# fuxiao0719/PanopticNeRF

Hardware: AMD Instinct MI355X
Metric: Msamples/sec (coarse+fine), KITTI-360 1408x376 (higher is better)
Workload: dtype bf16

## Files before the change

panopticnerf_amd/csrc/asm/gen_mlp_tt.py:

```python
#!/usr/bin/env python3
import os
import sys

if os.path.dirname(os.path.abspath(__file__)) not in sys.path:
    sys.path.insert(0, os.path.dirname(os.path.abspath(__file__)))
import tt_math
import tt_plan
from tt_emit import Emitter
from tt_regs import *



def vr(lo, n):
    return "v[%d:%d]" % (lo, lo + n - 1) if n > 1 else "v%d" % lo


def ar(lo, n):
    return "a[%d:%d]" % (lo, lo + n - 1) if n > 1 else "a%d" % lo


def sr(lo, n=2):
    return "s[%d:%d]" % (lo, lo + n - 1) if n > 1 else "s%d" % lo


# ... 26 lines not shown
        self.NC = len(self.chunks)
        self.units = tt_plan.build_units(self.layers, self.chunks)
        self.stream = []
        for u in self.units:
            u["frag0"] = len(self.stream)
            self.stream += [(sl, of) for sl, of, _, _ in self.unit_frags(u)]

    def unit_frags(self, u):
        return tt_plan.unit_frags(self.layers, self.chunks, u)

    def chunk_base(self, chunk):
        self.e("s_add_u32 s%d, s%d, 0x%x" % (S_PIECE, S_IMG, self.chunks[chunk]["off"] * 1024))
        self.e("s_addc_u32 s%d, s%d, 0" % (S_PIECE + 1, S_IMG + 1))

    def piece(self, chunk, j):
        m, i, nw = tt_plan.piece_list(self.chunks, chunk)[j]
        slot = chunk % NSLOT
        skip = None
        certain = nw >= 4
        if not certain:
            skip = self.label()
            self.e("s_cmp_ge_u32 s%d, %d" % (S_WAVE, nw))
            self.e("s_cbranch_scc1 %s" % skip)
        m0 = slot * SLOT + 16 * m * 1024
        if self.m0 != m0 or skip or self.trace:
            self.e("s_add_u32 m0, s%d, 0x%x" % (S_W4K, m0))
            self.e("s_nop 0")
        self.m0 = None if skip else m0
        tag = self.vm_op("global_load_lds_dwordx4 v%d, s[%d:%d] offset:%d" % (V_DMA + m, S_PIECE, S_PIECE + 1, i * 1024), certain)
        if skip:
            self.o.append(skip + ":")
        return tag

    def issue_piece(self, chunk, j):
        if j == 0:
            self.chunk_base(chunk)
        self.piece_tag[chunk] = self.piece(chunk, j)

    def hand_over(self, chunk):
        if not self.abl & 2:
            self.wait_vm(self.piece_tag.get((chunk + 2) % self.NC))
            self.e("s_barrier")

    def loc_of(self, seg, layer_index, t, ks):
        if seg == "ex":
            return Loc("v", V_EX + 16 * t + 4 * ks)
        if seg == "ed":
            return Loc("v", V_ED + 8 * t + 4 * ks)
        if seg == "h":
            src = self.trunk_out(layer_index - 1)
            return Loc("a", src + 64 * t + 4 * ks)
        if seg == "tap":
            return Loc("a", (self.F_base() if self.tap else self.trunk_out(D - 1)) + 64 * t + 4 * ks)
        if seg == "hh":
            return Loc("a", self.trunk_out(D - 1) + 64 * t + 4 * ks)
        if seg == "F":
            return Loc("a", self.F_base() + 64 * t + 4 * ks)
# ... 243 lines not shown

    def acc_reg(self, i):
        return V_ACC + 16 * i

    def acc_take(self, n):
        assert len(self.acc_free) >= n, ("accumulators exhausted", self.acc_free)
        got, self.acc_free = self.acc_free[:n], self.acc_free[n:]
        return got

    def acc_release(self, ids):
        self.acc_free = sorted(set(self.acc_free) | set(ids))

    def arm_plan(self, u):
        c = self.chunks[u["chunk"]]
        l = self.layers[u["layer"]]
        slot = u["chunk"] % NSLOT
        bias_off = c["nfb"] * l["nks"] * 1024
        u["accs"], u["arm_tags"] = {}, []
        plans = []
        for bi, blk in enumerate(u["blocks"]):
            b_in_chunk = blk - c["fb"]
            for t in range(2):
                key = (bi, t)
                ops = []

                def take(key=key):
                    while not self.acc_free and self.side_busy():
                        self.drain_side(8)
                    u["accs"][key] = self.acc_take(1)[0]
                if t == 1:
                    plans.append([take])
                    continue
                if l["mode"] == "logits":
                    def first(key=key, slot=slot, take=take):
                        take()
                        self.e("v_add_u32 v%d, 0x%x, v%d" % (self.acc_reg(u["accs"][key]), slot * SLOT, V_LB4))
                    ops.append(first)
                    for r in list(range(1, 16)) + [0]:
                        ops.append(lambda key=key, r=r, off=bias_off + b_in_chunk * 128: u["arm_tags"].append(
                            self.lgkm_op("ds_read_b32 v%d, v%d offset:%d" % (self.acc_reg(u["accs"][key]) + r, self.acc_reg(u["accs"][key]), off))))
                else:
                    for m in range(4):
                        def rd(key=key, m=m, off=bias_off + b_in_chunk * 128 + m * 32, take=take):
                            if m == 0:
                                take()
                            a = self.acc_reg(u["accs"][key])
                            u["arm_tags"].append(self.lgkm_op("ds_read_b128 %s, v%d offset:%d" % (vr(a + 4 * m, 4), V_BIAS + slot, off)))
                        ops.append(rd)
                plans.append(ops)
        return plans

    def pack_ops(self, u):
        l = self.layers[u["layer"]]
        if not self.trace:
            return self.pack_ops_pipelined(u)
        out = []
        for bi, blk in enumerate(u["blocks"]):
            for t in range(2):
                a = self.acc_reg(u["accs"][(bi, t)])
                dst = self.out_block(l, blk, t)
                for p in range(8):
                    def fn(a=a, p=p, dst=dst, relu=(l["mode"] == "relu"), k=len(out)):
# ... 312 lines not shown
                        a = self.acc_reg(u["accs"][(bi, t)])
                        dst = self.sm_sums[t][kk]
                        if r == 0:
                            e("v_fma_f32 v%d, v%d, v%d, 0" % (dst, M[t], a))
                        else:
                            e("v_fmac_f32 v%d, v%d, v%d" % (dst, M[t] + r, a + r))

    def lwr_ops(self):
        ops = []

        def first():
            while self.side or self.outbox or (len(self.acc_free) < 2 and self.side_busy()):
                self.drain_side(8)
            assert len(self.acc_free) >= 2, ("no free accumulators for the local weights", self.acc_free)
            self.lwr_acc = self.acc_take(2)
            self.e("v_add_u32 v%d, s%d, v%d" % (V_LWA, S_LWR, V_BIAS + 0))
        ops.append(first)
        for t in range(2):
            for q in range(4):
                for h2 in range(2):
                    def rd(t=t, q=q, h2=h2):
                        dst = self.acc_reg(self.lwr_acc[t]) + 4 * q + ((2 * h2 + 2) & 3)
                        self.lwr_tag = self.lgkm_op("ds_read_b64 %s, v%d offset:%d" % (vr(dst, 2), V_LWA, 128 * t + 32 * q + 8 * h2))
                    ops.append(rd)
        return ops

    def logit_blocks(self):
        return [(b, False) for b in range(self.nbs)] + [(0, True)] * self.nbi

    def tail_logits(self):
        e = self.e
# ... 135 lines not shown
        assert self.acc_free == [i for i in range(8) if i not in self.units[0]["accs"].values()], self.acc_free
        self.last_stamp = None
        for ui in range(len(self.units)):
            self.emit_unit(ui)
        self.stamp(len(self.units))
        self.drain_side()
        self.tail_logits()
        self.stamp(len(self.units) + 1)
        assert self.acc_free == list(range(8)), self.acc_free
        self.e("s_waitcnt lgkmcnt(0)")
        self.lgkm.drain()
        self.advance_group_state()
        self.stamp(len(self.units) + 2)
        if self.trace:
            self.o.append("\ts_waitcnt lgkmcnt(0)")
            self.stamp(len(self.units) + 3)

    def kernel(self):
        e, name = self.e, self.name
        self.o += ["\t.text", "\t.globl\t%s" % name, "\t.p2align\t8", "\t.type\t%s,@function" % name, "%s:" % name]
        for dst, off, n in ((S_IMG, 0x0, 2), (S_RAYS, 0x8, 2), (S_Z, 0x10, 2), (S_S, 0x18, 2), (S_MAGIC, 0x20, 2), (S_NGRP, 0x28, 2),
                            (S_REC, 0x30, 2), (S_RECF, 0x38, 1), (S_PS, 0x40, 2), (S_NSEM, 0x48, 2), (S_CLK, 0x50, 2), (S_AUX, 0x58, 2)):
            e("s_load_dword%s %s, %s, 0x%x" % ("x2" if n == 2 else "", sr(dst, n), sr(S_KARG), off))
        e("v_readfirstlane_b32 s%d, v0" % S_WAVE)
        e("s_nop 4")
        e("s_lshr_b32 s%d, s%d, 6" % (S_WAVE, S_WAVE))
        e("s_lshl_b32 s%d, s%d, 12" % (S_W4K, S_WAVE))
        e("v_and_b32 v%d, 63, v0" % V_T0)
        e("v_lshlrev_b32 v%d, 4, v%d" % (V_LANE16, V_T0))
        e("v_lshrrev_b32 v%d, 5, v0" % V_LB4)
        e("v_and_b32 v%d, 1, v%d" % (V_LB4, V_LB4))
        e("v_lshlrev_b32 v%d, 4, v%d" % (V_LB4, V_LB4))
        for sl in range(NSLOT):
            self.lit(S_T0, sl * SLOT)
            e("v_add_u32 v%d, s%d, v%d" % (V_FRAG + sl, S_T0, V_LANE16))
            e("v_add_u32 v%d, s%d, v%d" % (V_BIAS + sl, S_T0, V_LB4))
        for k in range(3):
            e("v_add_u32 v%d, s%d, v%d" % (V_DMA + k, S_W4K, V_LANE16))
            if k:
                e("v_add_u32 v%d, 0x%x, v%d" % (V_DMA + k, 16384 * k, V_DMA + k))
        e("v_and_b32 v%d, 31, v0" % V_LB4)
        e("v_lshlrev_b32 v%d, 2, v%d" % (V_LB4, V_LB4))
        e("s_mov_b32 s%d, -1" % S_LO32)
        e("s_mov_b32 s%d, 0" % (S_LO32 + 1))
        e("s_mov_b32 s%d, 1" % S_N0)
        e("s_mov_b32 s%d, 1" % (S_N0 + 1))
        e("s_mov_b32 s%d, -1" % S_HI0)
        e("s_mov_b32 s%d, 0" % (S_HI0 + 1))
        e("s_lshr_b32 s%d, s%d, 4" % (S_LWW, S_W4K))
        e("s_add_u32 s%d, s%d, 0x%x" % (S_LWW, S_LWW, LW_BASE))
        e("s_sub_u32 s%d, s%d, 0x%x" % (S_LWR, S_LWW, 0))
        e("s_waitcnt lgkmcnt(0)")
        for k, (blk, inst) in enumerate(self.logit_blocks()):
            e("v_and_b32 v%d, 31, v0" % V_T0)
            if blk:
                e("v_add_u32 v%d, %d, v%d" % (V_T0, 32 * blk, V_T0))
            e("v_cmp_gt_i32 vcc, s%d, v%d" % (S_NINST if inst else S_NSEM, V_T0))
            e("s_and_b64 s[%d:%d], vcc, s[%d:%d]" % (S_MSK + 2 * k, S_MSK + 2 * k + 1, S_HI0, S_HI0 + 1))
        if self.softmax:
            for k, (nblk, sreg) in enumerate(((self.nbs, S_NSEM), (self.nbi, S_NINST))):
                if nblk:
                    e("v_and_b32 v%d, 31, v0" % V_T0)
                    if nblk > 1:
                        e("v_add_u32 v%d, %d, v%d" % (V_T0, 32 * (nblk - 1), V_T0))
                    e("v_cmp_gt_i32 s[%d:%d], s%d, v%d" % (S_VMSK + 2 * k, S_VMSK + 2 * k + 1, sreg, V_T0))
        lend, lloop, lfin = self.label(), self.label(), self.label()
        e("s_mov_b32 s%d, s%d" % (S_GRP, S_WG))
        e("s_cmp_ge_i32 s%d, s%d" % (S_GRP, S_NGRP))
        e("s_cbranch_scc1 %s" % lend)
        for c in range(3):
            for j in range(tt_plan.pieces_of(self.chunks, c)):
                self.issue_piece(c, j)
        e("s_waitcnt vmcnt(0)")
        self.vm.drain()
        e("s_barrier")
        e("s_mov_b32 s%d, s%d" % (S_GRP2, S_GRP))
        tags = [self.fetch_tile(t, S_GRP2) for t in range(2)]
        for t in range(2):
            self.wait_vm(tags[t])
            for part in ("x", "d"):
                for fn in self.encode_tile(t, part):
                    fn()
        self.advance_group_state()
        if not self.trace:
            e("s_memtime s[%d:%d]" % (S_CLK0, S_CLK0 + 1))
            e("s_memrealtime s[%d:%d]" % (S_CLK0 + 2, S_CLK0 + 3))
        else:
            e("v_mov_b32 v%d, 0" % V_TRACE)
            e("s_mov_b32 s%d, 0" % S_NDONE)
            e("s_memtime %s" % sr(S_WGCLK))
            e("s_waitcnt lgkmcnt(0)")
        e("s_waitcnt lgkmcnt(0)")
        self.lgkm.drain()
        self.prefetch_first_unit()
        keep = self.o
        self.o = []
        self.group_body()
        self.prefetch_first_unit()
        self.o = keep
        self.o.append(lloop + ":")
        self.group_body()
        e("s_add_u32 s%d, s%d, s%d" % (S_GRP, S_GRP, S_NWG))
        e("s_cmp_ge_i32 s%d, s%d" % (S_GRP, S_NGRP))
        e("s_cbranch_scc1 %s" % lend)
# ... 10 lines not shown
            e("s_memtime s[%d:%d]" % (S_CLK0, S_CLK0 + 1))
            e("s_waitcnt lgkmcnt(0)")
            e("s_sub_u32 s%d, s%d, s%d" % (S_CLK0, S_CLK0, S_WGCLK))
            e("s_lshl_b32 s%d, s%d, 2" % (S_T0, S_WG))
            e("s_add_u32 s%d, s%d, 256" % (S_T0, S_T0))
            e("v_mov_b32 v%d, s%d" % (V_T0, S_T0))
            e("v_mov_b32 v%d, s%d" % (V_T1, S_CLK0))
            e("s_mov_b64 exec, 1")
            e("global_store_dword v%d, v%d, s[%d:%d]" % (V_T0, V_T1, S_CLK, S_CLK + 1))
            e("s_mov_b64 exec, -1")
            e("s_waitcnt vmcnt(0)")
            self.o.append(lw + ":")
        e("s_cmp_lg_u32 s%d, 0" % S_WG)
        e("s_cbranch_scc1 %s" % lfin)
        if self.trace:
            e("s_cmp_lg_u32 s%d, 0" % S_WAVE)
            e("s_cbranch_scc1 %s" % lfin)
            e("v_and_b32 v%d, 63, v0" % V_T0)
            e("v_lshlrev_b32 v%d, 2, v%d" % (V_T0, V_T0))
            e("global_store_dword v%d, v%d, s[%d:%d]" % (V_T0, V_TRACE, S_CLK, S_CLK + 1))
            e("s_waitcnt vmcnt(0)")
            e("s_branch %s" % lfin)
        e("s_memtime s[%d:%d]" % (S_T0, S_T0 + 1))
        e("s_memrealtime s[%d:%d]" % (S_SAVE, S_SAVE + 1))
        e("s_waitcnt lgkmcnt(0)")
        e("s_sub_u32 s%d, s%d, s%d" % (S_T0, S_T0, S_CLK0))
        e("s_subb_u32 s%d, s%d, s%d" % (S_T1, S_T1, S_CLK0 + 1))
        e("s_sub_u32 s%d, s%d, s%d" % (S_SAVE, S_SAVE, S_CLK0 + 2))
        e("s_subb_u32 s%d, s%d, s%d" % (S_SAVE + 1, S_SAVE + 1, S_CLK0 + 3))
        e("v_cmp_eq_u32 vcc, 0, v0")
        e("s_and_saveexec_b64 s[%d:%d], vcc" % (S_VALID, S_VALID + 1))
        e("s_cbranch_execz %s" % lfin)
        e("v_mov_b32 v%d, s%d" % (V_CLKOUT, S_T0))
        e("v_mov_b32 v%d, s%d" % (V_CLKOUT + 1, S_T1))
        e("v_mov_b32 v%d, s%d" % (V_CLKOUT + 2, S_SAVE))
        e("v_mov_b32 v%d, s%d" % (V_CLKOUT + 3, S_SAVE + 1))
        e("v_mov_b32 v%d, 0" % V_T0)
        e("global_store_dwordx4 v%d, %s, s[%d:%d]" % (V_T0, vr(V_CLKOUT, 4), S_CLK, S_CLK + 1))
        e("s_waitcnt vmcnt(0)")
        self.o.append(lfin + ":")
        e("s_endpgm")
        self.o += [".Lend_%s:" % name, "\t.size\t%s, .Lend_%s-%s" % (name, name, name), ""]
        self.o += ["\t.rodata", "\t.p2align\t6", "\t.amdhsa_kernel %s" % name,
                   "\t\t.amdhsa_group_segment_fixed_size %d" % (NSLOT * SLOT + 1024),
                   "\t\t.amdhsa_private_segment_fixed_size 0", "\t\t.amdhsa_kernarg_size %d" % KERNARG_BYTES, "\t\t.amdhsa_user_sgpr_count 2",
                   "\t\t.amdhsa_user_sgpr_kernarg_segment_ptr 1", "\t\t.amdhsa_system_sgpr_workgroup_id_x 1",
                   "\t\t.amdhsa_system_vgpr_workitem_id 0", "\t\t.amdhsa_next_free_vgpr 512", "\t\t.amdhsa_next_free_sgpr %d" % NEXT_FREE_SGPR,
                   "\t\t.amdhsa_accum_offset 256", "\t\t.amdhsa_reserve_vcc 1", "\t\t.amdhsa_float_denorm_mode_32 3",
                   "\t\t.amdhsa_float_denorm_mode_16_64 3", "\t\t.amdhsa_dx10_clamp 1", "\t\t.amdhsa_ieee_mode 1",
                   "\t.end_amdhsa_kernel", ""]
        return "\n".join(self.o)


KERNARG_BYTES = 104


def metadata(names):
    o = ["\t.amdgpu_metadata", "---", "amdhsa.kernels:"]
    for n in names:
        o += ["  - .agpr_count:     256", "    .args:", "      - .offset:         0", "        .size:           %d" % KERNARG_BYTES,
              "        .value_kind:     by_value", "    .group_segment_fixed_size: %d" % (NSLOT * SLOT + 1024),
              "    .kernarg_segment_align: 8", "    .kernarg_segment_size: %d" % KERNARG_BYTES, "    .max_flat_workgroup_size: 256",
              "    .name:           %s" % n, "    .private_segment_fixed_size: 0", "    .sgpr_count:     108",
              "    .sgpr_spill_count: 0", "    .symbol:         %s.kd" % n, "    .uniform_work_group_size: 1",
              "    .uses_dynamic_stack: false", "    .vgpr_count:     512", "    .vgpr_spill_count: 0", "    .wavefront_size: 64"]
    o += ["amdhsa.target:   amdgcn-amd-amdhsa--gfx950", "amdhsa.version:", "  - 1", "  - 2", "...", "\t.end_amdgpu_metadata", ""]
    return "\n".join(o)


def variant_name(tap, depth, sm, nbs, nbi):
    tag = ("f" if tap else "") + ("d1" if depth == 1 else "") + ("sm" if sm else "")
    return "k_mlp_tt_%ss%di%d" % (tag + "_" if tag else "", nbs, nbi)


def main():
    out = sys.argv[1] if len(sys.argv) > 1 else "/dev/stdout"
    parts = ['\t.amdgcn_target "amdgcn-amd-amdhsa--gfx950"', "\t.amdhsa_code_object_version 5", ""]
    names = []
    for nbs, nbi in ((1, 1), (2, 1), (0, 0), (1, 0), (2, 0), (3, 0)):
        n = "k_mlp_tt_s%di%d" % (nbs, nbi)
        names.append(n)
        parts.append(Gen(nbs, nbi, n).kernel())
    for tap in (0, 1):
        for depth in (2, 1):
            for sm in (False, True):
                if (tap, depth, sm) == (0, 2, False):
                    continue
                for nbs, nbi in ((1, 1), (2, 1), (1, 0), (2, 0), (3, 0)):
                    n = variant_name(tap, depth, sm, nbs, nbi)
                    names.append(n)
                    parts.append(Gen(nbs, nbi, n, depth=depth, softmax=sm, tap=tap).kernel())
    extra = sys.argv[3] if len(sys.argv) > 3 else ""
    if extra in ("trace", "abl"):
        names.append("k_mlp_tt_s2i1_trace")
        parts.append(Gen(2, 1, "k_mlp_tt_s2i1_trace", trace=True).kernel())
    if extra == "abl":
        for abl in (1, 2, 3, 4, 7):
            names.append("k_mlp_tt_s2i1_trace_a%d" % abl)
            parts.append(Gen(2, 1, names[-1], trace=True, abl=abl).kernel())
    unit_names = ["%s %s" % (g.layers[u["layer"]]["name"], u["blocks"]) for g in [Gen(2, 1, "x")] for u in g.units]
    if len(sys.argv) > 2:
        open(sys.argv[2], "w").write("\n".join(unit_names) + "\n")
    parts.append(metadata(names))
    with open(out, "w") as f:
        f.write("\n".join(parts))


if __name__ == "__main__":
    main()
```

panopticnerf_amd/csrc/asm/tt_plan.py:

```python
from tt_regs import D, NSLOT, SKIP


def build_plan(nbs, nbi, depth):
    L = []

    def add(name, nblk, segs, fbc, mode):
        nks = sum(n for _, n in segs)
        if fbc * nks + 1 > 33:
            fbc = 1
        L.append(dict(name=name, nblk=nblk, segs=segs, nks=nks, fbc=fbc, mode=mode))
    for i in range(D):
        if i == 0:
            add("L0", 8, [("ex", 4)], 8, "relu")
        elif i - 1 == SKIP:
            add("L%d" % i, 8, [("ex", 4), ("h", 16)], 2, "relu")
        else:
            add("L%d" % i, 8, [("h", 16)], 2, "relu")
    add("feature", 8, [("h", 16)], 2, "linear")
    add("views", 4, [("F", 16), ("ed", 2)], 2, "relu")
    add("rgbs", 1, [("g", 8), ("hh", 16)], 1, "rgbs")
    if depth == 1:
        if nbs:
            add("sem1", nbs, [("tap", 16)], nbs, "logits")
        if nbi:
            add("inst1", 1, [("tap", 16)], 1, "logits")
    else:
        if nbs:
            add("sem0", 4, [("tap", 16)], 2, "relu")
        if nbi:
            add("inst0", 4, [("tap", 16)], 2, "relu")
        if nbs:
            add("sem1", nbs, [("shs", 8)], nbs, "logits")
        if nbi:
            add("inst1", 1, [("shi", 8)], 1, "logits")
    chunks = []
    off = 0
    for li, l in enumerate(L):
        for fb in range(0, l["nblk"], l["fbc"]):
            nfrag = l["fbc"] * l["nks"] + 1
            chunks.append(dict(layer=li, fb=fb, nfb=l["fbc"], off=off, nfrag=nfrag))
            off += nfrag
    while len(chunks) % NSLOT:
        chunks.append(dict(layer=None, fb=0, nfb=0, off=0, nfrag=1, dummy=True))
    assert len(chunks) % NSLOT == 0, len(chunks)
    assert max(c["nfrag"] for c in chunks) <= 33
    return L, chunks


def build_units(layers, chunks):
    U = []
    for ci, c in enumerate(chunks):
        if c.get("dummy"):
            continue
        l = layers[c["layer"]]
        step = 2 if l["mode"] != "logits" else min(c["nfb"], 2)
        if l["name"] == "rgbs":
            step = 1
        blocks = list(range(c["fb"], c["fb"] + c["nfb"]))
        first = True
        for i in range(0, len(blocks), step):
            U.append(dict(chunk=ci, layer=c["layer"], blocks=blocks[i:i + step], first_of_chunk=first,
# ... 9 lines not shown
    for ks in range(l["nks"]):
        for bi, blk in enumerate(u["blocks"]):
            out.append((u["chunk"] % NSLOT, ((blk - c["fb"]) * l["nks"] + ks) * 1024, ks, bi))
    return out


def seg_of_ks(layer, ks):
    for seg, n in layer["segs"]:
        if ks < n:
            return seg, ks
        ks -= n
    raise IndexError


def piece_list(chunks, chunk):
    n = chunks[chunk]["nfrag"]
    out = []
    for m in range((n + 15) // 16):
        for i in range(4):
            nw = max(0, min(4, -(-(n - 16 * m - i) // 4)))
            if nw:
                out.append((m, i, nw))
    return out


def pieces_of(chunks, chunk):
    return len(piece_list(chunks, chunk))
```

panopticnerf_amd/csrc/asm/tt_regs.py:

```python

NSLOT, SLOT = 4, 33 * 1024
P = 4
D, SKIP = 8, 4
LW_BASE = NSLOT * SLOT

V_TID, V_LANE16, V_FRAG, V_BIAS, V_T0, V_DMA, V_LB4, V_TRACE = 0, 1, 2, 6, 10, 11, 14, 15
V_T1 = 1
V_T2 = 15
V_RING, V_ACC = 16, 32
V_CLKOUT = 20
V_EX, V_ED = 160, 192
V_G = 208
V_ZZ, V_ZN, V_DN, V_LW = 240, 242, 244, 246
V_IN = 224
V_TMP = 208
V_PTMP = 248
V_AUXA = V_PTMP + 6
V_LWA = V_IN + 2
V_SMX = V_IN + 10
A0, A1 = 0, 128
S_KARG, S_WG = 0, 2
S_IMG, S_RAYS, S_Z, S_S, S_N, S_MAGIC, S_SHIFT, S_NGRP, S_NWG, S_REC, S_RECF, S_PS, S_NSEM, S_NINST, S_CLK = 4, 6, 8, 10, 11, 12, 13, 14, 15, 16, 18, 20, 22, 23, 24
S_WAVE, S_W4K, S_GRP, S_PIECE, S_T0, S_T1 = 26, 27, 28, 30, 34, 35
S_VALID, S_LAST = 36, 40
S_NVALID, S_NLAST = 44, 48
S_LO32, S_N0, S_HI0 = 52, 54, 56
S_SAVE, S_REC_T = 58, 60
S_MSK = 64
S_REC_I = 70
S_AUX = 82
S_VMSK = 76
S_LWW, S_LWR = 74, 75
S_WGCLK = 90
S_CLK0 = 96
S_K = 100
S_NDONE = 101
S_Q = 19
S_GRP2 = 29

NEXT_FREE_SGPR = 102
TOPS = {"v": 256, "a": 256, "s": NEXT_FREE_SGPR}

RANGES = [
    ("v", "V_TID", V_TID, 1), ("v", "V_LANE16", V_LANE16, 1), ("v", "V_T1", V_T1, 1), ("v", "V_FRAG", V_FRAG, NSLOT),
    ("v", "V_BIAS", V_BIAS, NSLOT), ("v", "V_T0", V_T0, 1), ("v", "V_DMA", V_DMA, 3), ("v", "V_LB4", V_LB4, 1),
    ("v", "V_TRACE", V_TRACE, 1), ("v", "V_T2", V_T2, 1), ("v", "V_RING", V_RING, 4 * P), ("v", "V_CLKOUT", V_CLKOUT, 4),
    ("v", "V_ACC", V_ACC, 8 * 16), ("v", "V_EX", V_EX, 2 * 16), ("v", "V_ED", V_ED, 2 * 8), ("v", "V_G", V_G, 2 * 16),
    ("v", "V_TMP", V_TMP, 16), ("v", "V_IN", V_IN, 2 * 8), ("v", "V_LWA", V_LWA, 1), ("v", "V_SMX", V_SMX, 4),
    ("v", "V_ZZ", V_ZZ, 2), ("v", "V_ZN", V_ZN, 2), ("v", "V_DN", V_DN, 2), ("v", "V_LW", V_LW, 2),
    ("v", "V_PTMP", V_PTMP, 8), ("v", "V_AUXA", V_AUXA, 2),
    ("a", "A0", A0, 2 * 64), ("a", "A1", A1, 2 * 64),
    ("s", "S_KARG", S_KARG, 2), ("s", "S_WG", S_WG, 1), ("s", "S_IMG", S_IMG, 2), ("s", "S_RAYS", S_RAYS, 2), ("s", "S_Z", S_Z, 2),
    ("s", "S_S", S_S, 1), ("s", "S_N", S_N, 1), ("s", "S_MAGIC", S_MAGIC, 1), ("s", "S_SHIFT", S_SHIFT, 1), ("s", "S_NGRP", S_NGRP, 1),
    ("s", "S_NWG", S_NWG, 1), ("s", "S_REC", S_REC, 2), ("s", "S_RECF", S_RECF, 1), ("s", "S_Q", S_Q, 1), ("s", "S_PS", S_PS, 2),
    ("s", "S_NSEM", S_NSEM, 1), ("s", "S_NINST", S_NINST, 1), ("s", "S_CLK", S_CLK, 2), ("s", "S_WAVE", S_WAVE, 1),
    ("s", "S_W4K", S_W4K, 1), ("s", "S_GRP", S_GRP, 1), ("s", "S_GRP2", S_GRP2, 1), ("s", "S_PIECE", S_PIECE, 2),
    ("s", "S_T0", S_T0, 1), ("s", "S_T1", S_T1, 1), ("s", "S_VALID", S_VALID, 4), ("s", "S_LAST", S_LAST, 4),
    ("s", "S_NVALID", S_NVALID, 4), ("s", "S_NLAST", S_NLAST, 4), ("s", "S_LO32", S_LO32, 2), ("s", "S_N0", S_N0, 2),
    ("s", "S_HI0", S_HI0, 2), ("s", "S_SAVE", S_SAVE, 2), ("s", "S_REC_T", S_REC_T, 4), ("s", "S_MSK", S_MSK, 6),
    ("s", "S_REC_I", S_REC_I, 4), ("s", "S_LWW", S_LWW, 1), ("s", "S_LWR", S_LWR, 1), ("s", "S_VMSK", S_VMSK, 4),
    ("s", "S_AUX", S_AUX, 2), ("s", "S_WGCLK", S_WGCLK, 2), ("s", "S_CLK0", S_CLK0, 4), ("s", "S_K", S_K, 1),
    ("s", "S_NDONE", S_NDONE, 1),
]

OVERLAPS = [
    ("V_LANE16", "V_T1", "lane * 16 is only needed to build the bases in the prologue; the packs start behind it"),
    ("V_TRACE", "V_T2", "trace builds keep the plain pack form, which has no third temporary"),
    ("V_RING", "V_CLKOUT", "the clock store is the kernel's last: the fragment ring is idle"),
    ("V_G", "V_TMP", "encoder / epilogue temporaries share the g area once g is dead"),
    ("V_G", "V_IN", "views' packs of tile 1 land on the next group's inputs: what of them is live waits in an accumulator (Gen.park)"),
    ("V_G", "V_LWA", "inside V_IN; g is dead since the rgb / sigma unit"),
    ("V_G", "V_SMX", "inside V_IN; g is dead since the rgb / sigma unit"),
    ("V_IN", "V_LWA", "the next group's o_z: dead since its point"),
    ("V_IN", "V_SMX", "the next group's o_z and q of tile 1: dead once its gamma(d) is encoded"),
    ("V_PTMP", "V_AUXA", "the table address lives between the fetch of a tile and its point; the temporaries below it go on being used"),
]
# ... 23 lines not shown
```

panopticnerf_amd/csrc/pnr_mlp.hip:

```cpp
#include <stdlib.h>
#include <string.h>

#include "pnr_mlp_plan.h"

int pnr_mlp_validate(const pnr_mlp_desc* d);

#include "pnr_mlp_core.h"
#include "pnr_mlp_pp.h"
#include "pnr_mlp_fuse.h"
#include "pnr_mlp_tt.h"
#define PNR_QUERY_MAX_POINTS (((int64_t)1 << 31) - 4096)
template <int PREC, int TILES, class CTX, int KIND, int NA, int NB, int NFB_OUT, int MODE, int NOUT>
__device__ __forceinline__ void layer_regs(CTX& c, const uint32_t (&inA)[TILES][NA],
                                           const uint32_t (&inB)[TILES][NB > 0 ? NB : 1],
                                           uint32_t (&out)[TILES][NOUT], uint16_t* save = nullptr,
                                           const int* srow = nullptr)
{
    constexpr int RPB = PrecT<PREC>::RPB;
    constexpr int KS = NA / 4 + NB / 4;
    constexpr int FBC0 = pnr_layer_fbc(KIND, PREC);
    constexpr int FBC = (NFB_OUT % FBC0 == 0) ? FBC0 : 1;
    constexpr int G = (CTX::GDB / FBC) < 1 ? 1 : (CTX::GDB / FBC);
    static_assert(NOUT >= NFB_OUT * RPB, "output register array too small");
#pragma unroll
// ... 832 lines not shown
    a.rec = (float*)workspace;
    const int64_t tiles = ((int64_t)a.S + 255) / 256 * 8;
    a.ps = (float4*)(a.rec + tiles * a.rec_floats);
    hipStream_t st = (hipStream_t)stream;
    const bool softmax = (desc->flags & PNR_MLP_SOFTMAX) && desc->n_sem + desc->n_inst > 0;
    if (desc->plan == 3)
        return desc->W == 256 ? launch_mlp_pp<256, false, true, 0, true>(a, st) : launch_mlp_pp<128, false, true, 0, true>(a, st);
    if (desc->plan == 2) {
        PnrTTArgs t;
        memset(&t, 0, sizeof(t));
        t.image = a.data; t.rays = rays; t.z = z; t.S = a.S; t.N = a.N; t.n_magic = a.n_magic; t.n_shift = a.n_shift;
        t.rec = a.rec; t.rec_floats = a.rec_floats; t.ps = a.ps; t.n_sem = a.n_sem; t.n_inst = a.n_inst; t.clk = a.clk;
        PNR_REQUIRE(n_rays < ((int64_t)1 << 24), "pnr_mlp_forward_composite: the two-tile kernel addresses 2^24 rays per launch");
        uint32_t* aux = (uint32_t*)(((uintptr_t)((uint8_t*)a.ps + (int64_t)a.S * 16 + 256) + PNR_RAY_AUX_BYTES - 1)
                                    & ~(uintptr_t)(PNR_RAY_AUX_BYTES - 1));
        k_ray_aux<<<dim3((unsigned)((2 * n_rays + 255) / 256)), dim3(256), 0, st>>>(rays, n_rays, aux);
        t.aux = aux;
        t.n_wg = (desc->flags >> 16) & 0x1FF;
        const bool trace = (desc->flags & 0xFF00) == PNR_MLP_TRACE;
        return pnr_mlp_tt_launch(t, (desc->n_sem + 31) / 32, (desc->n_inst + 31) / 32, a.head_depth, a.head_tap, softmax, st, trace,
                                 trace ? ((desc->flags >> 4) & 7) : 0);
    }
    if (desc->plan == 1) {
        const int nbs = (desc->n_sem + 31) / 32, nbi = (desc->n_inst + 31) / 32;
        switch (4 * nbs + nbi + (softmax ? 16 : 0)) {
        case 4: return launch_mlp_pp<256, false, true, 4>(a, st);
        case 5: return launch_mlp_pp<256, false, true, 5>(a, st);
        case 8: return launch_mlp_pp<256, false, true, 8>(a, st);
        case 9: return launch_mlp_pp<256, false, true, 9>(a, st);
        case 20: return launch_mlp_pp<256, false, true, 20>(a, st);
        case 21: return launch_mlp_pp<256, false, true, 21>(a, st);
        case 24: return launch_mlp_pp<256, false, true, 24>(a, st);
        case 25: return launch_mlp_pp<256, false, true, 25>(a, st);
        default: PNR_REQUIRE(false, "pnr_mlp_forward_composite: no plan-1 kernel for %d + %d logit blocks", nbs, nbi);
        }
    }
// ... 252 lines not shown
```

panopticnerf_amd/csrc/pnr_mlp_tt.cpp:

```cpp
#include <mutex>
#include <string>

#include "pnr_common.h"
#include "pnr_mlp_tt.h"

static const unsigned char k_co[] = {
#include "pnr_mlp_tt_co.inc"
};

namespace {
struct DevTable {
    hipModule_t mod = nullptr;
    hipFunction_t fn[8][4][2] = {};
    hipFunction_t fn_trace[8] = {};
    bool tried = false, ok = false;
};
DevTable g_tab[64];
std::mutex g_mu;
}

static int tt_table(DevTable*& out, int capturing = 0)
{
    int dev = 0;
    PNR_HIP(hipGetDevice(&dev));
// ... 38 lines not shown
int pnr_mlp_tt_prepare(void)
{
    DevTable* t = nullptr;
    return tt_table(t);
}

void pnr_mlp_tt_prepare_quiet(void)
{
    int n = 0;
    if (hipGetDeviceCount(&n) != hipSuccess || n <= 0) { (void)hipGetLastError(); return; }
    const std::string keep = pnr_last_error();
    DevTable* t = nullptr;
    if (tt_table(t) != PNR_OK) pnr_set_error("%s", keep.c_str());
}

int pnr_mlp_tt_launch(const PnrTTArgs& a, int nbs, int nbi, int head_depth, int head_tap, bool softmax, hipStream_t stream, bool trace, int trace_abl)
{
    PNR_REQUIRE(nbs >= 0 && nbs <= 3 && nbi >= 0 && nbi <= (nbs == 1 || nbs == 2 ? 1 : 0), "pnr_mlp_forward_composite: no two-tile kernel for %d + %d logit blocks", nbs, nbi);
    PNR_REQUIRE(a.S >= 1 && a.S < (1 << 28), "pnr_mlp_forward_composite: the two-tile kernel takes R*N < 2^28 samples per launch (got %d): "
                "render in chunks", a.S);
    DevTable* t = nullptr;
    hipStreamCaptureStatus cs = hipStreamCaptureStatusNone;
    PNR_HIP(hipStreamIsCapturing(stream, &cs));
    int rc = tt_table(t, cs != hipStreamCaptureStatusNone);
    if (rc != PNR_OK) return rc;
    hipFunction_t fn = t->fn[!nbs ? 0 : (head_tap ? 4 : 0) + (softmax ? 2 : 0) + (head_depth == 1 ? 1 : 0)][nbs][nbi];
    PNR_REQUIRE(fn, "pnr_mlp_tt: no kernel for %d + %d logit blocks at head_depth %d", nbs, nbi, head_depth);
    if (trace) {
        PNR_REQUIRE(head_depth != 1 && !softmax && !head_tap, "pnr_mlp_tt: the trace build exists for head_depth 2, head_tap 0, logits compositing");
        PNR_REQUIRE(nbs == 2 && nbi == 1 && a.clk, "pnr_mlp_tt: the trace build exists for 2 + 1 logit blocks and needs the clock buffer");
        fn = t->fn_trace[trace_abl & 7];
        PNR_REQUIRE(fn, "pnr_mlp_tt: PNR_MLP_TRACE%s%d is not in this library: the trace kernels are diagnostics builds "
                    "(make EXTRA_TT=trace, ablations EXTRA_TT=abl)", trace_abl & 7 ? " ablation " : " ", trace_abl & 7);
    }
    PnrTTArgs ka = a;
    const int cus = pnr_cu_count();
    ka.n_groups = (a.S + 255) / 256;
    const int cap = (a.n_wg > 0 && a.n_wg < cus) ? a.n_wg : cus;
    ka.n_wg = ka.n_groups < cap ? ka.n_groups : cap;
    size_t size = sizeof(ka);
    void* extra[] = {HIP_LAUNCH_PARAM_BUFFER_POINTER, &ka, HIP_LAUNCH_PARAM_BUFFER_SIZE, &size, HIP_LAUNCH_PARAM_END};
    PNR_HIP(hipModuleLaunchKernel(fn, (unsigned)ka.n_wg, 1, 1, 256, 1, 1, 0, stream, nullptr, extra));
    return PNR_OK;
}
```

panopticnerf_amd/csrc/pnr_mlp_tt.h:

```cpp
#pragma once
#include <hip/hip_runtime.h>
#include <stdint.h>

struct PnrTTArgs {
    const void* image;
    const float* rays;
    const float* z;
    int32_t S, N;
    uint32_t n_magic;
    int32_t n_shift;
    int32_t n_groups, n_wg;
    float* rec;
    int32_t rec_floats, pad0;
    void* ps;
    int32_t n_sem, n_inst;
    unsigned long long* clk;
    const void* aux;
    uint64_t reserved;
};
static_assert(sizeof(PnrTTArgs) == 104, "k_mlp_tt reads its arguments at fixed offsets");

int pnr_mlp_tt_prepare(void);
void pnr_mlp_tt_prepare_quiet(void);
int pnr_mlp_tt_launch(const PnrTTArgs& a, int nbs, int nbi, int head_depth, int head_tap, bool softmax, hipStream_t stream, bool trace = false,
                      int trace_abl = 0);
```

Before: 1158.

## Preload bias table into LDS once and balance weight-fragment DMA across waves

Biases are now copied into a dedicated LDS bias table once per workgroup at kernel start, instead of travelling as an extra fragment with every weight chunk into the ring slots. Each chunk's per-wave global_load_lds pieces are re-split so the four waves get balanced fragment counts, with new per-k wave offset registers, and dummy chunks are pinned to specific waves. This is meant to cut the per-chunk DMA volume and the wait imbalance before each barrier, at the cost of more LDS and extra setup registers. The host side also resolves the kernel before launching k_ray_aux and adds trace-only barrier-time counters.

```diff
diff --git a/panopticnerf_amd/csrc/asm/gen_mlp_tt.py b/panopticnerf_amd/csrc/asm/gen_mlp_tt.py
--- a/panopticnerf_amd/csrc/asm/gen_mlp_tt.py
+++ b/panopticnerf_amd/csrc/asm/gen_mlp_tt.py
@@ -64,23 +64,52 @@
         self.e("s_addc_u32 s%d, s%d, 0" % (S_PIECE + 1, S_IMG + 1))
 
     def piece(self, chunk, j):
-        m, i, nw = tt_plan.piece_list(self.chunks, chunk)[j]
+        m, i, nw, k, w0 = tt_plan.piece_list(self.chunks, chunk)[j]
         slot = chunk % NSLOT
         skip = None
         certain = nw >= 4
         if not certain:
+            assert w0 == 0 or nw == 1
             skip = self.label()
-            self.e("s_cmp_ge_u32 s%d, %d" % (S_WAVE, nw))
+            self.e("s_cmp_ge_u32 s%d, %d" % (S_WAVE, nw) if w0 == 0 else "s_cmp_lg_u32 s%d, %d" % (S_WAVE, w0))
             self.e("s_cbranch_scc1 %s" % skip)
+        if k == 4:
+            v_off, s_wave = V_DMA + m, S_W4K
+        else:
+            v_off, s_wave = V_DMAT + DMAT[k, m], S_WKK + k - 1
         m0 = slot * SLOT + 16 * m * 1024
-        if self.m0 != m0 or skip or self.trace:
-            self.e("s_add_u32 m0, s%d, 0x%x" % (S_W4K, m0))
+        if self.m0 != (s_wave, m0) or skip or self.trace:
+            self.e("s_add_u32 m0, s%d, 0x%x" % (s_wave, m0))
             self.e("s_nop 0")
-        self.m0 = None if skip else m0
-        tag = self.vm_op("global_load_lds_dwordx4 v%d, s[%d:%d] offset:%d" % (V_DMA + m, S_PIECE, S_PIECE + 1, i * 1024), certain)
+        self.m0 = None if skip else (s_wave, m0)
+        tag = self.vm_op("global_load_lds_dwordx4 v%d, s[%d:%d] offset:%d" % (v_off, S_PIECE, S_PIECE + 1, i * 1024), certain)
         if skip:
             self.o.append(skip + ":")
         return tag
+
+    def lds_bytes(self):
+        n = BT_BASE + tt_plan.bias_table_bytes(self.chunks)
+        assert n <= LDS_TOP, n
+        return n
+
+    def fill_bias_table(self):
+        e = self.e
+        loads = tt_plan.bias_table_loads(self.chunks)
+        assert all(0 <= dst and dst + BT_LOAD <= self.lds_bytes() - BT_BASE for _, dst in loads)
+        e("v_and_b32 v%d, 63, v0" % V_T0)
+        e("v_lshlrev_b32 v%d, 2, v%d" % (V_T0, V_T0))
+        for w in range(4):
+            nxt = self.label()
+            e("s_cmp_lg_u32 s%d, %d" % (S_WAVE, w))
+            e("s_cbranch_scc1 %s" % nxt)
+            for src, dst in loads[w::4]:
+                e("s_add_u32 s%d, s%d, 0x%x" % (S_PIECE, S_IMG, src))
+                e("s_addc_u32 s%d, s%d, 0" % (S_PIECE + 1, S_IMG + 1))
+                e("s_mov_b32 m0, 0x%x" % (BT_BASE + dst))
+                e("s_nop 0")
+                e("global_load_lds_dword v%d, s[%d:%d]" % (V_T0, S_PIECE, S_PIECE + 1))
+            self.o.append(nxt + ":")
+        self.m0 = None
 
     def issue_piece(self, chunk, j):
         if j == 0:
@@ -90,7 +119,19 @@
     def hand_over(self, chunk):
         if not self.abl & 2:
             self.wait_vm(self.piece_tag.get((chunk + 2) % self.NC))
+            if self.trace:
+                self.bar_sum()
+                self.o.append("\ts_memtime %s" % sr(S_BAR))
+                self.o.append("\ts_barrier")
+                self.o.append("\ts_memtime %s" % sr(S_BAR + 2))
+                return
             self.e("s_barrier")
+
+    def bar_sum(self):
+        self.o.append("\ts_sub_u32 s%d, s%d, s%d" % (S_BAR, S_BAR + 2, S_BAR))
+        self.o.append("\ts_add_u32 s%d, s%d, s%d" % (S_BW, S_BW, S_BAR))
+        self.o.append("\ts_mov_b32 s%d, 0" % S_BAR)
+        self.o.append("\ts_mov_b32 s%d, 0" % (S_BAR + 2))
 
     def loc_of(self, seg, layer_index, t, ks):
         if seg == "ex":
@@ -364,8 +405,7 @@
     def arm_plan(self, u):
         c = self.chunks[u["chunk"]]
         l = self.layers[u["layer"]]
-        slot = u["chunk"] % NSLOT
-        bias_off = c["nfb"] * l["nks"] * 1024
+        bias_off = c["bt"]
         u["accs"], u["arm_tags"] = {}, []
         plans = []
         for bi, blk in enumerate(u["blocks"]):
@@ -382,9 +422,9 @@
                     plans.append([take])
                     continue
                 if l["mode"] == "logits":
-                    def first(key=key, slot=slot, take=take):
+                    def first(key=key, take=take):
                         take()
-                        self.e("v_add_u32 v%d, 0x%x, v%d" % (self.acc_reg(u["accs"][key]), slot * SLOT, V_LB4))
+                        self.e("v_add_u32 v%d, 0x%x, v%d" % (self.acc_reg(u["accs"][key]), BT_BASE, V_LB4))
                     ops.append(first)
                     for r in list(range(1, 16)) + [0]:
                         ops.append(lambda key=key, r=r, off=bias_off + b_in_chunk * 128: u["arm_tags"].append(
@@ -395,7 +435,7 @@
                             if m == 0:
                                 take()
                             a = self.acc_reg(u["accs"][key])
-                            u["arm_tags"].append(self.lgkm_op("ds_read_b128 %s, v%d offset:%d" % (vr(a + 4 * m, 4), V_BIAS + slot, off)))
+                            u["arm_tags"].append(self.lgkm_op("ds_read_b128 %s, v%d offset:%d" % (vr(a + 4 * m, 4), V_BIAS, off)))
                         ops.append(rd)
                 plans.append(ops)
         return plans
@@ -738,7 +778,7 @@
                 self.drain_side(8)
             assert len(self.acc_free) >= 2, ("no free accumulators for the local weights", self.acc_free)
             self.lwr_acc = self.acc_take(2)
-            self.e("v_add_u32 v%d, s%d, v%d" % (V_LWA, S_LWR, V_BIAS + 0))
+            self.e("v_add_u32 v%d, s%d, v%d" % (V_LWA, S_LWR, V_BIAS))
         ops.append(first)
         for t in range(2):
             for q in range(4):
@@ -904,6 +944,9 @@
         self.stamp(len(self.units) + 2)
         if self.trace:
             self.o.append("\ts_waitcnt lgkmcnt(0)")
+            self.bar_sum()
+            self.o.append("\ts_mov_b32 s%d, s%d" % (S_BW + 1, S_BW))
+            self.o.append("\ts_mov_b32 s%d, 0" % S_BW)
             self.stamp(len(self.units) + 3)
 
     def kernel(self):
@@ -924,11 +967,17 @@
         for sl in range(NSLOT):
             self.lit(S_T0, sl * SLOT)
             e("v_add_u32 v%d, s%d, v%d" % (V_FRAG + sl, S_T0, V_LANE16))
-            e("v_add_u32 v%d, s%d, v%d" % (V_BIAS + sl, S_T0, V_LB4))
-        for k in range(3):
+        e("v_add_u32 v%d, 0x%x, v%d" % (V_BIAS, BT_BASE, V_LB4))
+        for k in range(2):
             e("v_add_u32 v%d, s%d, v%d" % (V_DMA + k, S_W4K, V_LANE16))
             if k:
                 e("v_add_u32 v%d, 0x%x, v%d" % (V_DMA + k, 16384 * k, V_DMA + k))
+        for k in (1, 2):
+            e("s_lshl_b32 s%d, s%d, %d" % (S_WKK + k - 1, S_WAVE, 9 + k))
+        for (k, m), r in sorted(DMAT.items()):
+            e("v_add_u32 v%d, s%d, v%d" % (V_DMAT + r, S_WKK + k - 1, V_LANE16))
+            if m:
+                e("v_add_u32 v%d, 0x%x, v%d" % (V_DMAT + r, 16384 * m, V_DMAT + r))
         e("v_and_b32 v%d, 31, v0" % V_LB4)
         e("v_lshlrev_b32 v%d, 2, v%d" % (V_LB4, V_LB4))
         e("s_mov_b32 s%d, -1" % S_LO32)
@@ -939,7 +988,7 @@
         e("s_mov_b32 s%d, 0" % (S_HI0 + 1))
         e("s_lshr_b32 s%d, s%d, 4" % (S_LWW, S_W4K))
         e("s_add_u32 s%d, s%d, 0x%x" % (S_LWW, S_LWW, LW_BASE))
-        e("s_sub_u32 s%d, s%d, 0x%x" % (S_LWR, S_LWW, 0))
+        e("s_sub_u32 s%d, s%d, 0x%x" % (S_LWR, S_LWW, BT_BASE))
         e("s_waitcnt lgkmcnt(0)")
         for k, (blk, inst) in enumerate(self.logit_blocks()):
             e("v_and_b32 v%d, 31, v0" % V_T0)
@@ -958,6 +1007,7 @@
         e("s_mov_b32 s%d, s%d" % (S_GRP, S_WG))
         e("s_cmp_ge_i32 s%d, s%d" % (S_GRP, S_NGRP))
         e("s_cbranch_scc1 %s" % lend)
+        self.fill_bias_table()
         for c in range(3):
             for j in range(tt_plan.pieces_of(self.chunks, c)):
                 self.issue_piece(c, j)
@@ -978,6 +1028,9 @@
         else:
             e("v_mov_b32 v%d, 0" % V_TRACE)
             e("s_mov_b32 s%d, 0" % S_NDONE)
+            for k in (0, 2):
+                e("s_mov_b32 s%d, 0" % (S_BAR + k))
+            e("s_mov_b64 %s, 0" % sr(S_BW))
             e("s_memtime %s" % sr(S_WGCLK))
             e("s_waitcnt lgkmcnt(0)")
         e("s_waitcnt lgkmcnt(0)")
@@ -1018,6 +1071,19 @@
         e("s_cmp_lg_u32 s%d, 0" % S_WG)
         e("s_cbranch_scc1 %s" % lfin)
         if self.trace:
+            for w in (1, 2):
+                e("s_cmp_eq_u32 s%d, %d" % (S_WAVE, w))
+                e("s_cbranch_scc1 %s" % lfin)
+            e("s_lshr_b32 s%d, s%d, 1" % (S_T0, S_WAVE))
+            e("s_add_u32 s%d, s%d, s%d" % (S_T0, S_T0, S_NWG))
+            e("s_add_u32 s%d, s%d, 64" % (S_T0, S_T0))
+            e("s_lshl_b32 s%d, s%d, 2" % (S_T0, S_T0))
+            e("v_mov_b32 v%d, s%d" % (V_T0, S_T0))
+            e("v_mov_b32 v%d, s%d" % (V_T1, S_BW + 1))
+            e("s_mov_b64 exec, 1")
+            e("global_store_dword v%d, v%d, s[%d:%d]" % (V_T0, V_T1, S_CLK, S_CLK + 1))
+            e("s_mov_b64 exec, -1")
+            e("s_waitcnt vmcnt(0)")
             e("s_cmp_lg_u32 s%d, 0" % S_WAVE)
             e("s_cbranch_scc1 %s" % lfin)
             e("v_and_b32 v%d, 63, v0" % V_T0)
@@ -1046,7 +1112,7 @@
         e("s_endpgm")
         self.o += [".Lend_%s:" % name, "\t.size\t%s, .Lend_%s-%s" % (name, name, name), ""]
         self.o += ["\t.rodata", "\t.p2align\t6", "\t.amdhsa_kernel %s" % name,
-                   "\t\t.amdhsa_group_segment_fixed_size %d" % (NSLOT * SLOT + 1024),
+                   "\t\t.amdhsa_group_segment_fixed_size %d" % self.lds_bytes(),
                    "\t\t.amdhsa_private_segment_fixed_size 0", "\t\t.amdhsa_kernarg_size %d" % KERNARG_BYTES, "\t\t.amdhsa_user_sgpr_count 2",
                    "\t\t.amdhsa_user_sgpr_kernarg_segment_ptr 1", "\t\t.amdhsa_system_sgpr_workgroup_id_x 1",
                    "\t\t.amdhsa_system_vgpr_workitem_id 0", "\t\t.amdhsa_next_free_vgpr 512", "\t\t.amdhsa_next_free_sgpr %d" % NEXT_FREE_SGPR,
@@ -1059,11 +1125,11 @@
 KERNARG_BYTES = 104
 
 
-def metadata(names):
+def metadata(names, lds):
     o = ["\t.amdgpu_metadata", "---", "amdhsa.kernels:"]
     for n in names:
         o += ["  - .agpr_count:     256", "    .args:", "      - .offset:         0", "        .size:           %d" % KERNARG_BYTES,
-              "        .value_kind:     by_value", "    .group_segment_fixed_size: %d" % (NSLOT * SLOT + 1024),
+              "        .value_kind:     by_value", "    .group_segment_fixed_size: %d" % lds[n],
               "    .kernarg_segment_align: 8", "    .kernarg_segment_size: %d" % KERNARG_BYTES, "    .max_flat_workgroup_size: 256",
               "    .name:           %s" % n, "    .private_segment_fixed_size: 0", "    .sgpr_count:     108",
               "    .sgpr_spill_count: 0", "    .symbol:         %s.kd" % n, "    .uniform_work_group_size: 1",
@@ -1080,32 +1146,31 @@
 def main():
     out = sys.argv[1] if len(sys.argv) > 1 else "/dev/stdout"
     parts = ['\t.amdgcn_target "amdgcn-amd-amdhsa--gfx950"', "\t.amdhsa_code_object_version 5", ""]
-    names = []
+    names, lds = [], {}
+
+    def add(g):
+        names.append(g.name)
+        lds[g.name] = g.lds_bytes()
+        parts.append(g.kernel())
     for nbs, nbi in ((1, 1), (2, 1), (0, 0), (1, 0), (2, 0), (3, 0)):
-        n = "k_mlp_tt_s%di%d" % (nbs, nbi)
-        names.append(n)
-        parts.append(Gen(nbs, nbi, n).kernel())
+        add(Gen(nbs, nbi, "k_mlp_tt_s%di%d" % (nbs, nbi)))
     for tap in (0, 1):
         for depth in (2, 1):
             for sm in (False, True):
                 if (tap, depth, sm) == (0, 2, False):
                     continue
                 for nbs, nbi in ((1, 1), (2, 1), (1, 0), (2, 0), (3, 0)):
-                    n = variant_name(tap, depth, sm, nbs, nbi)
-                    names.append(n)
-                    parts.append(Gen(nbs, nbi, n, depth=depth, softmax=sm, tap=tap).kernel())
+                    add(Gen(nbs, nbi, variant_name(tap, depth, sm, nbs, nbi), depth=depth, softmax=sm, tap=tap))
     extra = sys.argv[3] if len(sys.argv) > 3 else ""
     if extra in ("trace", "abl"):
-        names.append("k_mlp_tt_s2i1_trace")
-        parts.append(Gen(2, 1, "k_mlp_tt_s2i1_trace", trace=True).kernel())
+        add(Gen(2, 1, "k_mlp_tt_s2i1_trace", trace=True))
     if extra == "abl":
         for abl in (1, 2, 3, 4, 7):
-            names.append("k_mlp_tt_s2i1_trace_a%d" % abl)
-            parts.append(Gen(2, 1, names[-1], trace=True, abl=abl).kernel())
+            add(Gen(2, 1, "k_mlp_tt_s2i1_trace_a%d" % abl, trace=True, abl=abl))
     unit_names = ["%s %s" % (g.layers[u["layer"]]["name"], u["blocks"]) for g in [Gen(2, 1, "x")] for u in g.units]
     if len(sys.argv) > 2:
         open(sys.argv[2], "w").write("\n".join(unit_names) + "\n")
-    parts.append(metadata(names))
+    parts.append(metadata(names, lds))
     with open(out, "w") as f:
         f.write("\n".join(parts))
 
diff --git a/panopticnerf_amd/csrc/asm/tt_plan.py b/panopticnerf_amd/csrc/asm/tt_plan.py
--- a/panopticnerf_amd/csrc/asm/tt_plan.py
+++ b/panopticnerf_amd/csrc/asm/tt_plan.py
@@ -1,4 +1,4 @@
-from tt_regs import D, NSLOT, SKIP
+from tt_regs import BT_LOAD, D, NSLOT, SKIP
 
 
 def build_plan(nbs, nbi, depth):
@@ -34,17 +34,32 @@
         if nbi:
             add("inst1", 1, [("shi", 8)], 1, "logits")
     chunks = []
-    off = 0
+    off = bt = 0
     for li, l in enumerate(L):
         for fb in range(0, l["nblk"], l["fbc"]):
             nfrag = l["fbc"] * l["nks"] + 1
-            chunks.append(dict(layer=li, fb=fb, nfb=l["fbc"], off=off, nfrag=nfrag))
+            chunks.append(dict(layer=li, fb=fb, nfb=l["fbc"], off=off, nfrag=nfrag, nwf=nfrag - 1, bt=bt))
             off += nfrag
+            bt += -(-l["fbc"] * 128 // BT_LOAD) * BT_LOAD
     while len(chunks) % NSLOT:
-        chunks.append(dict(layer=None, fb=0, nfb=0, off=0, nfrag=1, dummy=True))
+        chunks.append(dict(layer=None, fb=0, nfb=0, off=0, nfrag=1, nwf=1, dummy=True))
     assert len(chunks) % NSLOT == 0, len(chunks)
-    assert max(c["nfrag"] for c in chunks) <= 33
+    assert max(c["nfrag"] for c in chunks) <= 33 and max(c["nwf"] for c in chunks) <= 32
+    check_balance(chunks)
     return L, chunks
+
+
+def bias_table_bytes(chunks):
+    return max(c["bt"] + -(-c["nfb"] * 128 // BT_LOAD) * BT_LOAD for c in chunks if not c.get("dummy"))
+
+
+def bias_table_loads(chunks):
+    out = []
+    for c in chunks:
+        if not c.get("dummy"):
+            for k in range(-(-c["nfb"] * 128 // BT_LOAD)):
+                out.append(((c["off"] + c["nwf"]) * 1024 + k * BT_LOAD, c["bt"] + k * BT_LOAD))
+    return out
 
 
 def build_units(layers, chunks):
@@ -84,15 +99,33 @@
 
 
 def piece_list(chunks, chunk):
-    n = chunks[chunk]["nfrag"]
+    n = chunks[chunk]["nwf"]
+    if chunks[chunk].get("dummy"):
+        return [(0, 0, 1, 4, 2 + chunk % 2)]
     out = []
     for m in range((n + 15) // 16):
-        for i in range(4):
-            nw = max(0, min(4, -(-(n - 16 * m - i) // 4)))
-            if nw:
-                out.append((m, i, nw))
+        r = min(16, n - 16 * m)
+        k = -(-r // 4)
+        for i in range(k):
+            nw = sum(1 for w in range(4) if k * w + i < r)
+            out.append((m, i, nw, k, 0))
     return out
 
 
 def pieces_of(chunks, chunk):
     return len(piece_list(chunks, chunk))
+
+
+def pieces_per_wave(chunks, chunk):
+    return [sum(1 for _, _, nw, _, w0 in piece_list(chunks, chunk) if w0 <= w < w0 + nw) for w in range(4)]
+
+
+def check_balance(chunks):
+    tot = [0] * 4
+    for ci, c in enumerate(chunks):
+        per = pieces_per_wave(chunks, ci)
+        assert max(per) - min(per) <= (1 if c["nwf"] % 4 else 0), (ci, c["nwf"], per)
+        assert sum(per) == c["nwf"], (ci, per)
+        tot = [a + b for a, b in zip(tot, per)]
+    assert (max(tot) - min(tot)) * 50 <= max(tot), tot
+    return tot
diff --git a/panopticnerf_amd/csrc/asm/tt_regs.py b/panopticnerf_amd/csrc/asm/tt_regs.py
--- a/panopticnerf_amd/csrc/asm/tt_regs.py
+++ b/panopticnerf_amd/csrc/asm/tt_regs.py
@@ -3,8 +3,11 @@
 P = 4
 D, SKIP = 8, 4
 LW_BASE = NSLOT * SLOT
+BT_BASE, BT_LOAD = LW_BASE + 1024, 256
+LDS_TOP = 160 * 1024
 
-V_TID, V_LANE16, V_FRAG, V_BIAS, V_T0, V_DMA, V_LB4, V_TRACE = 0, 1, 2, 6, 10, 11, 14, 15
+V_TID, V_LANE16, V_FRAG, V_BIAS, V_DMAT, V_T0, V_DMA, V_LB4, V_TRACE = 0, 1, 2, 6, 7, 10, 11, 14, 15
+DMAT = {(1, 1): 0, (2, 0): 1, (2, 1): 2}
 V_T1 = 1
 V_T2 = 15
 V_RING, V_ACC = 16, 32
@@ -21,7 +24,7 @@
 A0, A1 = 0, 128
 S_KARG, S_WG = 0, 2
 S_IMG, S_RAYS, S_Z, S_S, S_N, S_MAGIC, S_SHIFT, S_NGRP, S_NWG, S_REC, S_RECF, S_PS, S_NSEM, S_NINST, S_CLK = 4, 6, 8, 10, 11, 12, 13, 14, 15, 16, 18, 20, 22, 23, 24
-S_WAVE, S_W4K, S_GRP, S_PIECE, S_T0, S_T1 = 26, 27, 28, 30, 34, 35
+S_WAVE, S_W4K, S_GRP, S_PIECE, S_WKK, S_T0, S_T1 = 26, 27, 28, 30, 32, 34, 35
 S_VALID, S_LAST = 36, 40
 S_NVALID, S_NLAST = 44, 48
 S_LO32, S_N0, S_HI0 = 52, 54, 56
@@ -32,6 +35,7 @@
 S_VMSK = 76
 S_LWW, S_LWR = 74, 75
 S_WGCLK = 90
+S_BAR, S_BW = 84, 88
 S_CLK0 = 96
 S_K = 100
 S_NDONE = 101
@@ -43,7 +47,7 @@
 
 RANGES = [
     ("v", "V_TID", V_TID, 1), ("v", "V_LANE16", V_LANE16, 1), ("v", "V_T1", V_T1, 1), ("v", "V_FRAG", V_FRAG, NSLOT),
-    ("v", "V_BIAS", V_BIAS, NSLOT), ("v", "V_T0", V_T0, 1), ("v", "V_DMA", V_DMA, 3), ("v", "V_LB4", V_LB4, 1),
+    ("v", "V_BIAS", V_BIAS, 1), ("v", "V_DMAT", V_DMAT, len(DMAT)), ("v", "V_T0", V_T0, 1), ("v", "V_DMA", V_DMA, 2), ("v", "V_LB4", V_LB4, 1),
     ("v", "V_TRACE", V_TRACE, 1), ("v", "V_T2", V_T2, 1), ("v", "V_RING", V_RING, 4 * P), ("v", "V_CLKOUT", V_CLKOUT, 4),
     ("v", "V_ACC", V_ACC, 8 * 16), ("v", "V_EX", V_EX, 2 * 16), ("v", "V_ED", V_ED, 2 * 8), ("v", "V_G", V_G, 2 * 16),
     ("v", "V_TMP", V_TMP, 16), ("v", "V_IN", V_IN, 2 * 8), ("v", "V_LWA", V_LWA, 1), ("v", "V_SMX", V_SMX, 4),
@@ -54,12 +58,12 @@
     ("s", "S_S", S_S, 1), ("s", "S_N", S_N, 1), ("s", "S_MAGIC", S_MAGIC, 1), ("s", "S_SHIFT", S_SHIFT, 1), ("s", "S_NGRP", S_NGRP, 1),
     ("s", "S_NWG", S_NWG, 1), ("s", "S_REC", S_REC, 2), ("s", "S_RECF", S_RECF, 1), ("s", "S_Q", S_Q, 1), ("s", "S_PS", S_PS, 2),
     ("s", "S_NSEM", S_NSEM, 1), ("s", "S_NINST", S_NINST, 1), ("s", "S_CLK", S_CLK, 2), ("s", "S_WAVE", S_WAVE, 1),
-    ("s", "S_W4K", S_W4K, 1), ("s", "S_GRP", S_GRP, 1), ("s", "S_GRP2", S_GRP2, 1), ("s", "S_PIECE", S_PIECE, 2),
+    ("s", "S_W4K", S_W4K, 1), ("s", "S_GRP", S_GRP, 1), ("s", "S_GRP2", S_GRP2, 1), ("s", "S_PIECE", S_PIECE, 2), ("s", "S_WKK", S_WKK, 2),
     ("s", "S_T0", S_T0, 1), ("s", "S_T1", S_T1, 1), ("s", "S_VALID", S_VALID, 4), ("s", "S_LAST", S_LAST, 4),
     ("s", "S_NVALID", S_NVALID, 4), ("s", "S_NLAST", S_NLAST, 4), ("s", "S_LO32", S_LO32, 2), ("s", "S_N0", S_N0, 2),
     ("s", "S_HI0", S_HI0, 2), ("s", "S_SAVE", S_SAVE, 2), ("s", "S_REC_T", S_REC_T, 4), ("s", "S_MSK", S_MSK, 6),
     ("s", "S_REC_I", S_REC_I, 4), ("s", "S_LWW", S_LWW, 1), ("s", "S_LWR", S_LWR, 1), ("s", "S_VMSK", S_VMSK, 4),
-    ("s", "S_AUX", S_AUX, 2), ("s", "S_WGCLK", S_WGCLK, 2), ("s", "S_CLK0", S_CLK0, 4), ("s", "S_K", S_K, 1),
+    ("s", "S_AUX", S_AUX, 2), ("s", "S_WGCLK", S_WGCLK, 2), ("s", "S_BAR", S_BAR, 4), ("s", "S_BW", S_BW, 2), ("s", "S_CLK0", S_CLK0, 4), ("s", "S_K", S_K, 1),
     ("s", "S_NDONE", S_NDONE, 1),
 ]
 
diff --git a/panopticnerf_amd/csrc/pnr_mlp.hip b/panopticnerf_amd/csrc/pnr_mlp.hip
--- a/panopticnerf_amd/csrc/pnr_mlp.hip
+++ b/panopticnerf_amd/csrc/pnr_mlp.hip
@@ -870,12 +870,16 @@
         PNR_REQUIRE(n_rays < ((int64_t)1 << 24), "pnr_mlp_forward_composite: the two-tile kernel addresses 2^24 rays per launch");
         uint32_t* aux = (uint32_t*)(((uintptr_t)((uint8_t*)a.ps + (int64_t)a.S * 16 + 256) + PNR_RAY_AUX_BYTES - 1)
                                     & ~(uintptr_t)(PNR_RAY_AUX_BYTES - 1));
-        k_ray_aux<<<dim3((unsigned)((2 * n_rays + 255) / 256)), dim3(256), 0, st>>>(rays, n_rays, aux);
         t.aux = aux;
         t.n_wg = (desc->flags >> 16) & 0x1FF;
         const bool trace = (desc->flags & 0xFF00) == PNR_MLP_TRACE;
-        return pnr_mlp_tt_launch(t, (desc->n_sem + 31) / 32, (desc->n_inst + 31) / 32, a.head_depth, a.head_tap, softmax, st, trace,
-                                 trace ? ((desc->flags >> 4) & 7) : 0);
+        PnrTTKernel k;
+        rc = pnr_mlp_tt_resolve(t, (desc->n_sem + 31) / 32, (desc->n_inst + 31) / 32, a.head_depth, a.head_tap, softmax, st, trace,
+                                trace ? ((desc->flags >> 4) & 7) : 0, k);
+        if (rc != PNR_OK) return rc;
+        k_ray_aux<<<dim3((unsigned)((2 * n_rays + 255) / 256)), dim3(256), 0, st>>>(rays, n_rays, aux);
+        PNR_CHECK_LAUNCH("pnr_mlp_forward_composite (k_ray_aux)");
+        return pnr_mlp_tt_launch(t, k, st);
     }
     if (desc->plan == 1) {
         const int nbs = (desc->n_sem + 31) / 32, nbi = (desc->n_inst + 31) / 32;
diff --git a/panopticnerf_amd/csrc/pnr_mlp_tt.cpp b/panopticnerf_amd/csrc/pnr_mlp_tt.cpp
--- a/panopticnerf_amd/csrc/pnr_mlp_tt.cpp
+++ b/panopticnerf_amd/csrc/pnr_mlp_tt.cpp
@@ -76,7 +76,8 @@
     if (tt_table(t) != PNR_OK) pnr_set_error("%s", keep.c_str());
 }
 
-int pnr_mlp_tt_launch(const PnrTTArgs& a, int nbs, int nbi, int head_depth, int head_tap, bool softmax, hipStream_t stream, bool trace, int trace_abl)
+int pnr_mlp_tt_resolve(const PnrTTArgs& a, int nbs, int nbi, int head_depth, int head_tap, bool softmax, hipStream_t stream, bool trace,
+                       int trace_abl, PnrTTKernel& out)
 {
     PNR_REQUIRE(nbs >= 0 && nbs <= 3 && nbi >= 0 && nbi <= (nbs == 1 || nbs == 2 ? 1 : 0), "pnr_mlp_forward_composite: no two-tile kernel for %d + %d logit blocks", nbs, nbi);
     PNR_REQUIRE(a.S >= 1 && a.S < (1 << 28), "pnr_mlp_forward_composite: the two-tile kernel takes R*N < 2^28 samples per launch (got %d): "
@@ -95,6 +96,14 @@
         PNR_REQUIRE(fn, "pnr_mlp_tt: PNR_MLP_TRACE%s%d is not in this library: the trace kernels are diagnostics builds "
                     "(make EXTRA_TT=trace, ablations EXTRA_TT=abl)", trace_abl & 7 ? " ablation " : " ", trace_abl & 7);
     }
+    out.fn = fn;
+    return PNR_OK;
+}
+
+int pnr_mlp_tt_launch(const PnrTTArgs& a, const PnrTTKernel& k, hipStream_t stream)
+{
+    PNR_REQUIRE(k.fn, "pnr_mlp_tt_launch: no kernel resolved");
+    hipFunction_t fn = (hipFunction_t)k.fn;
     PnrTTArgs ka = a;
     const int cus = pnr_cu_count();
     ka.n_groups = (a.S + 255) / 256;
diff --git a/panopticnerf_amd/csrc/pnr_mlp_tt.h b/panopticnerf_amd/csrc/pnr_mlp_tt.h
--- a/panopticnerf_amd/csrc/pnr_mlp_tt.h
+++ b/panopticnerf_amd/csrc/pnr_mlp_tt.h
@@ -22,5 +22,7 @@
 
 int pnr_mlp_tt_prepare(void);
 void pnr_mlp_tt_prepare_quiet(void);
-int pnr_mlp_tt_launch(const PnrTTArgs& a, int nbs, int nbi, int head_depth, int head_tap, bool softmax, hipStream_t stream, bool trace = false,
-                      int trace_abl = 0);
+struct PnrTTKernel { void* fn = nullptr; };
+int pnr_mlp_tt_resolve(const PnrTTArgs& a, int nbs, int nbi, int head_depth, int head_tap, bool softmax, hipStream_t stream, bool trace,
+                       int trace_abl, PnrTTKernel& out);
+int pnr_mlp_tt_launch(const PnrTTArgs& a, const PnrTTKernel& k, hipStream_t stream);
```

New measurement: 1168 (median of 6 runs). No clear change (+0.9%).
